# UzL-ITS/dash

Hardware: AMD Instinct MI355X
Metric: online garbled inferences/sec (MiniONN CIFAR-10 CNN) (higher is better)
Workload: dtype uint8 label components / int8 MFMA (exact modular arithmetic)

## Files before the change

### dash_amd/csrc/hip/gadget_common.h

```cpp
#pragma once

#include <cmath>
#include <cstdio>
#include <cstdlib>

#include "kargs.h"
#include "launch.h"

namespace dash {
namespace dev {

constexpr size_t kAesLds = 0;

#ifndef DASH_AES_BLOCK
#define DASH_AES_BLOCK 512
#endif
constexpr int kAesBlock = DASH_AES_BLOCK;
#ifndef DASH_AES_MINBLOCKS
#define DASH_AES_MINBLOCKS 6
#endif
constexpr int kAesMinBlocks = DASH_AES_MINBLOCKS;
#ifndef DASH_SA_MINBLOCKS
#define DASH_SA_MINBLOCKS 6
#endif
constexpr int kSignApproxMinWaves = DASH_SA_MINBLOCKS;
#ifndef DASH_SA_CHUNK
#define DASH_SA_CHUNK 16
#endif
constexpr int kSignApproxChunk = DASH_SA_CHUNK;

static int aes_block_cap(int bs) {
    const int waves = std::max(kAesMinBlocks, kSignApproxMinWaves);
    const int resident = std::max(1, std::min(waves * 256 / bs, 160 * 1024 / DASH_AES_LDS_BYTES));
    return 4 * resident * num_cus();
}
static inline dim3 grid_aes(int64_t n, int bs, int y, int z) {
    int64_t nx = (n + bs - 1) / bs;
    const int64_t capx = std::max<int64_t>(1, aes_block_cap(bs) / (static_cast<int64_t>(y) * z));
    return dim3(static_cast<unsigned>(std::min(nx, capx)), y, z);
}
static inline int aes_bs(int64_t n, int y, int z) {
    const int64_t lanes = n * y * z;
    int bs = kAesBlock;
    while (bs > 64 && lanes < static_cast<int64_t>(bs) * num_cus()) bs >>= 1;
    return bs;
}
struct LaunchDims {
    dim3 grid, block;
};
static inline LaunchDims aes_dims(const char* kernel, int64_t n, int y, int z) {
    const int bs = aes_bs(n, y, z);
    const LaunchDims d{grid_aes(n, bs, y, z), dim3(bs)};
    if (launch_log_on()) {
        std::string name(kernel);
        if (!name.empty() && name.front() == '(') name = name.substr(1, name.size() - 2);
        launch_log_add("aes." + name, d.grid, d.block);
    }
    return d;
}
#define AES_LAUNCH_GGL(kernel, n, y, z, lds, st, ...)                        \
    do {                                                                     \
        const LaunchDims d_ = aes_dims(#kernel, (n), (y), (z));              \
        hipLaunchKernelGGL(kernel, d_.grid, d_.block, lds, st, __VA_ARGS__); \
    } while (0)

#define AES_PROLOGUE(tab, rk)                    \
    __shared__ __attribute__((aligned(16))) uint32_t lds_aes[DASH_AES_LDS_WORDS]; \
    aes_lds_fill(lds_aes, tab);                   \
    const AesCtx aes = aes_ctx(lds_aes, rk)

template <int BS, int U, bool ZERO = false>
__device__ __forceinline__ void lds_stage_rows(uint8_t* S, const act_t* L, int64_t N, int64_t e0, int c0, int cnt) {
    constexpr int W = BS / 16;
    const int units = cnt * W;
    for (int x0 = threadIdx.x; x0 < units; x0 += U * BS) {
        uint4 v[U];
#pragma unroll
        for (int h = 0; h < U; ++h) {
            const int x = x0 + h * BS;
            const int64_t e = e0 + 16 * (x % W);
            if constexpr (ZERO) v[h] = make_uint4(0u, 0u, 0u, 0u);
            if (x < units && e < N) v[h] = *reinterpret_cast<const uint4*>(L + static_cast<int64_t>(c0 + x / W) * N + e);
        }
#pragma unroll
        for (int h = 0; h < U; ++h) {
            const int x = x0 + h * BS;
            if (x < units) *reinterpret_cast<uint4*>(S + (x / W) * BS + 16 * (x % W)) = v[h];
        }
    }
}
template <int BS>
__device__ __forceinline__ void lds_store_rows(act_t* L, const uint8_t* S, int64_t N, int64_t e0, int c0, int cnt) {
    constexpr int W = BS / 16;
    const int units = cnt * W;
    for (int x = threadIdx.x; x < units; x += BS) {
        const int64_t e = e0 + 16 * (x % W);
        if (e < N)
            *reinterpret_cast<uint4*>(L + static_cast<int64_t>(c0 + x / W) * N + e) =
                *reinterpret_cast<const uint4*>(S + (x / W) * BS + 16 * (x % W));
    }
}
static inline bool stage_ok(int64_t N, int bs) {
    static const bool on = [] {
        const char* e = std::getenv("DASH_MRS_STAGE");
        return !(e && e[0] == '0');
    }();
    return on && N % 16 == 0 && N >= bs;
}

#ifndef DASH_UA_MINBLOCKS
#define DASH_UA_MINBLOCKS 4
#endif

template <int CTRL>
__device__ __forceinline__ u128 dpp128(u128 v) {
    const uint32_t w0 = static_cast<uint32_t>(__builtin_amdgcn_mov_dpp(static_cast<int>(static_cast<uint32_t>(v)), CTRL, 0xF, 0xF, false));
    const uint32_t w1 = static_cast<uint32_t>(__builtin_amdgcn_mov_dpp(static_cast<int>(static_cast<uint32_t>(v >> 32)), CTRL, 0xF, 0xF, false));
    const uint32_t w2 = static_cast<uint32_t>(__builtin_amdgcn_mov_dpp(static_cast<int>(static_cast<uint32_t>(v >> 64)), CTRL, 0xF, 0xF, false));
    const uint32_t w3 = static_cast<uint32_t>(__builtin_amdgcn_mov_dpp(static_cast<int>(static_cast<uint32_t>(v >> 96)), CTRL, 0xF, 0xF, false));
    return (static_cast<u128>((static_cast<uint64_t>(w3) << 32) | w2) << 64) | ((static_cast<uint64_t>(w1) << 32) | w0);
}
__device__ __forceinline__ u128 quad_sum128(u128 v) {
    v += dpp128<0xB1>(v);
    return v + dpp128<0x4E>(v);
}
struct QPow {
    u128 d1, d2, d3, d4;
    __device__ __forceinline__ void init(const ModC& m) {
        d1 = static_cast<u128>(m.D);
        d2 = d1 * d1;
        d3 = d2 * d1;
        d4 = d2 * d2;
    }
    __device__ __forceinline__ u128 first(int g) const {
        return g == 0 ? static_cast<u128>(1) : (g == 1 ? d1 : (g == 2 ? d2 : d3));
    }
};

}
}
```

### dash_amd/csrc/hip/launch.h

```cpp
#pragma once

#include <hip/hip_runtime.h>

#include <algorithm>
#include <atomic>
#include <cstdlib>
#include <map>
#include <mutex>
#include <string>
#include <vector>

#include "kargs.h"

namespace dash {
namespace dev {

int num_cus();
void set_planning_cus(int n);
int planning_cus_override();
int64_t joint_fuse_min_elems();
int joint_fuse_mode();
void set_joint_fuse(int mode);
bool joint_fuse_pick(int64_t N, int B);
bool joint_fuse(int64_t N, int B);
bool leaky_fuse(int64_t N, int B);
bool clip_fuse_pick(int64_t N, int B);
bool clip_fuse(int64_t N, int B);
constexpr int kConstModDefault = 1;
int const_mod_mode();
void set_const_mod(int mode);
inline bool const_mod_on() { return const_mod_mode() >= 1; }
inline bool const_mod_chain() { return const_mod_mode() >= 2; }
void const_mod_count(bool chain);
long const_mod_launches(bool chain);
constexpr int kChainFpK = 7;
inline bool chain_const_mod_pick(const int* p, int k) {
    if (k != kChainFpK) return false;
    for (int r = 0; r < k; ++r)
        if (p[r] != static_cast<int>(kFirstPrimes[r])) return false;
    return true;
}
extern std::atomic<bool> g_launch_log_on;
inline bool launch_log_on() { return g_launch_log_on.load(std::memory_order_relaxed); }
void launch_log_enable(bool on);
void launch_log_add(const std::string& form, dim3 grid, dim3 block);
std::vector<std::string> launch_log_take();


void launch_sign_approx(const SignArgs& a, const Act& x, const ModC* mc, const AesGlobals& g, hipStream_t st);
void launch_sign_chain(const SignArgs& a, int maxn, const ModC* mc, const AesGlobals& g, hipStream_t st);
void launch_unpack(const u128* P, int nres, const Act& out, const CrtInfo& mods, const ModC* mc, int64_t N, int B,
                   hipStream_t st);
void launch_clip_hash(const ClipArgs& a, u128* hx, uint16_t* colx, const Act& x, int B, const ModC* mc,
                      const AesGlobals& g, hipStream_t st);
void launch_clip_sign_mrs(const MrsArgs& a, const Act& x, int B, const ModC* mc, const AesGlobals& g, hipStream_t st);
void launch_clip_mult(const ClipArgs& a, const Act& x, const Act& y, int B, const ModC* mc, hipStream_t st);
void launch_argmax_diff(const Act& v, const Act& d, int64_t P, int ops, int cnt, int pubq, const CrtInfo& crt, int B,
                        hipStream_t st);
void launch_argmax_hash(const Act& d, const CrtInfo& crt, int64_t N, u128* hx, uint16_t* colx, uint64_t gate0, int B,
                        const ModC* mc, const AesGlobals& g, hipStream_t st);
void launch_argmax_mult(const ArgMaxArgs& a, bool val, bool l0, const Act& v, const Act& d, const Act& i, const Act& ed,
                        const Act& nv, const Act& ni, int B, const ModC* mc, hipStream_t st);
void launch_pwl_key(const PwlArgs& a, u128* kx, uint16_t* colx, const Act& x, int B, const ModC* mc, hipStream_t st);
void launch_pwl_mult(const PwlArgs& a, const Act& x, const Act& y, int B, const ModC* mc, hipStream_t st);
void launch_leaky_mult(const SignArgs& a, const LeakyTab& lk, const Act& x, const Act& y, const u128* gtab,
                       const u128* etab, const ModC* mc, hipStream_t st);
void launch_leaky_mrs(const MrsArgs& a, const SignArgs& sa, const LeakyTab& lk, const Act& x, const Act& y,
                      const u128* gtab, const u128* etab, int B, const ModC* mc, const AesGlobals& g, hipStream_t st);
void launch_rescale_leaky_out(const MrsArgs& a, const SignArgs& sa, const LeakyTab& lk, const Act& x, const Act& y,
                              const u128* gtab, const u128* etab, int B, const ModC* mc, const AesGlobals& g,
                              hipStream_t st);
void launch_relu_mult(const SignArgs& a, const Act& x, const Act& y, const u128* gtab, const u128* etab,
                      const ModC* mc, hipStream_t st);
void launch_rescale_hash(const Act& x, int fi, int s, const int16_t* up, int up_stride, int add_up, int64_t N, int B,
                         u128* h0, uint16_t* col0, const ModC* mc, const AesGlobals& g, hipStream_t st, int hard = 0);
void launch_rescale_update(const RescaleArgs& a, const Act& x, int B, const ModC* mc, hipStream_t st);
void launch_rescale_post(const Act& x, const CrtInfo& crt, int64_t N, int B, const u128* signP, const int16_t* down,
                         int lab_stride, const int* lab_off, const ModC* mc, hipStream_t st);
void launch_rescale_hash_sign(const u128* signP, const u128* du, int64_t N, int B, u128* h0, uint16_t* col0,
                              const AesGlobals& g, hipStream_t st);
void launch_rescale_update_approx(const RescaleArgs& r, const SignArgs& a, const Act& x, const int16_t* delta,
                                  const u128* zh, int B, const ModC* mc, const AesGlobals& g, hipStream_t st);
void launch_rescale_mrs(const MrsArgs& a, const Act& x, int B, const ModC* mc, const AesGlobals& g, hipStream_t st,
                        bool chain_only = false);
void launch_rescale_mrs_out(const MrsArgs& a, const Act& x, int B, const ModC* mc, const AesGlobals& g,
                            hipStream_t st);
template <int K>
void launch_mrs_chain_k(const MrsArgs& a, const Act& x, int B, const ModC* mc, const AesGlobals& g, hipStream_t st);
void launch_rescale_relu_out(const MrsArgs& a, const SignArgs& sa, const Act& x, const Act& y, const u128* gtab,
                             const u128* etab, int B, const ModC* mc, const AesGlobals& g, hipStream_t st);
void launch_rescale_clip_out(const MrsArgs& a, const ClipArgs& ca, const Act& x, const Act& y, int B, const ModC* mc,
                             const AesGlobals& g, hipStream_t st);
void launch_relu_joint(const SignArgs& sa, const Act& x, const Act& y, const u128* gtab, const u128* etab, int B,
                       const ModC* mc, const AesGlobals& g, hipStream_t st);
void launch_relu_mrs(const MrsArgs& a, const SignArgs& sa, const Act& x, const Act& y, const u128* gtab,
                     const u128* etab, int B, const ModC* mc, const AesGlobals& g, hipStream_t st);
void launch_base_ext(const BEArgs& a, const Act& x, int B, const ModC* mc, const AesGlobals& g, hipStream_t st);
void launch_proj(const ProjArgs& a, const Act& x, const Act& y, int B, const ModC* mc, const AesGlobals& g,
                 hipStream_t st);
void launch_mul(const MulArgs& a, bool square, const Act& x, const Act& ys, const Act& y, int B, const ModC* mc,
                hipStream_t st);
void launch_label_key(const CrtInfo& crt, int64_t N, u128* kx, uint16_t* colx, const Act& x, int B, const ModC* mc,
                      hipStream_t st);
void launch_matmul(const MatMulArgs& a, const Act& y, int B, const ModC* mc, hipStream_t st);
void launch_mult(const MultArgs& a, const Act& x, const Act& y, int B, const ModC* mc, const AesGlobals& g,
                 hipStream_t st);

void launch_copy_gather(const Act& in, int64_t Nin, const Act& out, int64_t Nout, const int64_t* idx,
                        const CrtInfo& crt, int B, hipStream_t st);
void launch_gather(const Act& in, int64_t Nin, const Act& out, int64_t Nout, const int32_t* idx4, const int64_t* idx8,
                   const CrtInfo& crt, int B, hipStream_t st);
struct BilinearArgs {
    int C, H, W, OH, OW, OWp;
    const int2* rows;
    const int2* cols;
    const uint16_t* wrow;
    const uint16_t* wcol;
    uint32_t mq[kMaxRes];
};
struct BilinearTables {
    std::vector<int2> rows, cols;
    std::vector<uint16_t> wrow, wcol;
};
template <class Geom>
BilinearTables bilinear_tables(BilinearArgs& a, const Geom& G, const int* mods, int k) {
    a.C = static_cast<int>(G.C); a.H = static_cast<int>(G.H); a.W = static_cast<int>(G.W);
    a.OH = static_cast<int>(G.OH); a.OW = static_cast<int>(G.OW);
    a.OWp = (a.OW + 3) / 4 * 4;
    BilinearTables t;
    t.rows.resize(static_cast<size_t>(a.OH));
    t.cols.assign(static_cast<size_t>(a.OWp), make_int2(0, 0));
    t.wrow.resize(static_cast<size_t>(k) * a.OH);
    t.wcol.assign(static_cast<size_t>(k) * a.OWp, 0);
    for (int oy = 0; oy < a.OH; ++oy)
        t.rows[oy] = make_int2(static_cast<int>((*G.y0)[oy]), static_cast<int>((*G.y1)[oy]));
    for (int ox = 0; ox < a.OW; ++ox)
        t.cols[ox] = make_int2(static_cast<int>((*G.x0)[ox]), static_cast<int>((*G.x1)[ox]));
    for (int j = 0; j < k; ++j) {
        const int p = mods[j];
        a.mq[j] = static_cast<uint32_t>((uint64_t(1) << 32) / static_cast<uint64_t>(p));
        for (int oy = 0; oy < a.OH; ++oy)
            t.wrow[static_cast<size_t>(j) * a.OH + oy] = static_cast<uint16_t>(G.wy(oy, 0, p) | G.wy(oy, 1, p) << 8);
        for (int ox = 0; ox < a.OW; ++ox)
            t.wcol[static_cast<size_t>(j) * a.OWp + ox] = static_cast<uint16_t>(G.wx(ox, 0, p) | G.wx(ox, 1, p) << 8);
    }
    return t;
}
void launch_bilinear(const BilinearArgs& g, bool dword, const Act& in, const Act& out, const CrtInfo& crt, int B,
                     hipStream_t st);
void launch_pair_diff(const Act& v, int64_t Nv, const Act& d, int64_t Nout, int ops, int cnt, const CrtInfo& crt, int B,
                      hipStream_t st);
void launch_pair_add(const Act& v, int64_t Nv, const Act& r, const Act& nv, int64_t Nout, int ops, int cnt, int cnt1,
                     const CrtInfo& crt, int B, hipStream_t st);
void launch_add(const Act& x, const Act& y, int64_t N, const CrtInfo& crt, int B, hipStream_t st);
void launch_window_sum(const Act& in, int64_t Nin, const Act& out, int64_t Nout, const int64_t* idx, int K,
                       const CrtInfo& crt, int B, hipStream_t st);
struct PoolArgs {
    int C, H, W, kh, kw, sh, sw, ph, pw, OH, OW;
};
void launch_pool_sum(const Act& in, const Act& out, const PoolArgs& g, const CrtInfo& crt, int B, hipStream_t st);
void launch_concat_copy(const Act& src, int64_t Ns, const Act& out, int64_t Nout, int64_t off, const CrtInfo& crt,
                        int B, hipStream_t st);
void launch_aes_bench(u128* out, int blocks, int iters, const AesGlobals& g, hipStream_t st);
void launch_aes_test(const u128* in, u128* out, int64_t n, const AesGlobals& g, hipStream_t st);
void launch_hard_test(const u128* key, const uint64_t* gate, const uint32_t* sub, const uint32_t* blk, u128* out,
                      int64_t n, hipStream_t st);
constexpr int kModkTestRow = 64;
void launch_modk_test(int q, const uint32_t* r, int64_t N, uint32_t* out, hipStream_t st);
void launch_codec_test(const int16_t* labels, int64_t N, int q, const ModC* mc, u128* comp, int16_t* decomp,
                       hipStream_t st);

struct DenseArgs {
    CrtInfo crt;
    int64_t K, O;
    const int16_t* w[kMaxRes];
    const int32_t* zc[kMaxRes];
    const int16_t* bias[kMaxRes];
    const int16_t* zero;
    int lab_stride;
    int lab_off[kMaxRes];
    const int32_t* src;
// ... 300 lines not shown
```

### dash_amd/csrc/hip/mrs_chain.h

```cpp
#pragma once

#include "gadget_common.h"

namespace dash {
namespace dev {

__device__ __forceinline__ u128 add_packed(u128 a, u128 b, u128 hmask) {
    return ((a & ~hmask) + (b & ~hmask)) ^ ((a ^ b) & hmask);
}

#ifndef DASH_MRS_CHUNK
#define DASH_MRS_CHUNK 4
#endif
constexpr int kMrsChunk = DASH_MRS_CHUNK;
#ifndef DASH_MRS_M2CH
#define DASH_MRS_M2CH 16
#endif
template <int K>
__device__ __forceinline__ constexpr int mrs_pair(int l, int j) {
    return l * (2 * K - l - 1) / 2 + (j - l - 1);
}

template <int MODE>
__device__ __forceinline__ constexpr uint32_t mrs_row_sub(int i) {
    return tw_sub(MODE == 1 ? kTwSmrs : kTwMrs, static_cast<uint32_t>(i));
}
__device__ __forceinline__ void store_ypads(const MrsArgs& a, u128 key, int b, int64_t N, int64_t e) {
    const uint64_t g = a.rgate0 ^ static_cast<uint64_t>(e);
    for (int blk = 0; 4 * blk < a.ny; ++blk) {
        u128 p[4];
        hard_block(key, g, tw_sub(kTwMmy, 0), static_cast<uint32_t>(blk), p);
#pragma unroll
        for (int q = 0; q < 4; ++q)
            if (4 * blk + q < a.ny) a.ys[(static_cast<int64_t>(b) * a.ny + 4 * blk + q) * N + e] = p[q];
    }
}

template <int MODE>
__device__ __forceinline__ void store_sign_key(const MrsArgs& a, u128 key, int b, int64_t N, int64_t e) {
    if (MODE >= 1 && a.ks) a.ks[static_cast<int64_t>(b) * N + e] = key;
}

#ifndef DASH_CHAIN2_WAVES
#define DASH_CHAIN2_WAVES 4
#endif
template <int K, int MODE>
__global__ __launch_bounds__(kAesBlock, MODE == 2 ? DASH_CHAIN2_WAVES : DASH_UA_MINBLOCKS) void k_mrs_chain(MrsArgs a, Act x, const ModC* mc,
                                                                          const uint32_t* te0, const uint32_t* rk) {
    (void)te0;
    (void)rk;
    const int b = blockIdx.z;
    const int64_t N = a.N;
    constexpr int NP = K * (K - 1) / 2 > 0 ? K * (K - 1) / 2 : 1;
    for (int64_t e = static_cast<int64_t>(blockIdx.x) * blockDim.x + threadIdx.x; e < N;
         e += static_cast<int64_t>(gridDim.x) * blockDim.x) {
        const u128* row0 = a.tab + (static_cast<int64_t>(b) * N + e) * a.n_tab;
        u128* PS = a.ps + static_cast<int64_t>(b) * NP * N + e;
        u128 acc = 0;
#pragma unroll
        for (int i = 0; i < (MODE >= 1 ? K - 1 : K); ++i) {
            const int r = MODE >= 1 ? (i + 1) % K : i;
            const ModC m = mc[a.crt.p[r]];
            const int n = static_cast<int>(m.n);
            const act_t* L = x.p[r] + static_cast<int64_t>(b) * n * N + e;
            DigitStream ds[K > 1 ? K - 1 : 1];
#pragma unroll
            for (int l = 0; l < i; ++l) ds[l].init(PS[static_cast<int64_t>(mrs_pair<K>(l, i)) * N]);
            CompressFwd cf;
            cf.init();
            uint32_t col = 0;
            uint16_t cur[kMrsChunk], nxt[kMrsChunk];
#pragma unroll
            for (int u = 0; u < kMrsChunk; ++u)
                if (u < n) cur[u] = static_cast<uint16_t>(L[static_cast<int64_t>(u) * N]);
            for (int c0 = 0; c0 < n; c0 += kMrsChunk) {
#pragma unroll
                for (int u = 0; u < kMrsChunk; ++u)
                    if (c0 + kMrsChunk + u < n) nxt[u] = static_cast<uint16_t>(L[static_cast<int64_t>(c0 + kMrsChunk + u) * N]);
#pragma unroll
                for (int u = 0; u < kMrsChunk; ++u)
                    if (c0 + u < n) {
                        uint32_t d = cur[u];
#pragma unroll
                        for (int l = 0; l < i; ++l) {
                            const uint32_t s = ds[l].next(m);
                            d = d >= s ? d - s : d + m.q - s;
                        }
                        if (c0 + u == 0) col = d;
                        cf.push(d, m);
                    }
#pragma unroll
                for (int u = 0; u < kMrsChunk; ++u) cur[u] = nxt[u];
            }
            constexpr int kExtra = MODE == 1 ? 0 : 1;
            const int nt = K - 1 - i + kExtra;
            const u128* row = row0 + a.dig_off[i] + static_cast<int64_t>(col) * nt;
            u128 E[K];
#pragma unroll
            for (int t = 0; t < nt; ++t) E[t] = row[t];
            hard_unmask_n<K>(E, nt, cf.finish(), a.gate0 ^ static_cast<uint64_t>(e), mrs_row_sub<MODE>(i));
#pragma unroll
            for (int t = 0; t < K - 1 - i; ++t) PS[static_cast<int64_t>(mrs_pair<K>(i, i + 1 + t)) * N] = E[t];
            if (MODE != 1) acc = add_packed(acc, E[K - 1 - i], a.hmask);
        }
        if (MODE >= 1) {
            const ModC m = mc[a.crt.p[0]];
            const act_t* L = x.p[0] + static_cast<int64_t>(b) * m.n * N + e;
            u128 key = compress_cm<DASH_MRS_M2CH>(L, N, m);
#pragma unroll
            for (int l = 0; l < K - 1; ++l) key ^= PS[static_cast<int64_t>(mrs_pair<K>(l, K - 1)) * N];
            const uint32_t c = static_cast<uint32_t>(key) & 1u;
            u128 E = 0;
            if (MODE == 2)
                E = row0[a.dig_off[K - 1] + c] - hard_pad(key, a.gate0 ^ static_cast<uint64_t>(e), mrs_row_sub<MODE>(K - 1), 0);
            store_ypads(a, key, b, N, e);
            store_sign_key<MODE>(a, key, b, N, e);
            a.cs[static_cast<int64_t>(b) * N + e] = static_cast<uint8_t>(c);
            if (MODE == 2) acc = add_packed(acc, E, a.hmask);
        }
        if (MODE == 1) continue;
        const uint32_t col = static_cast<uint32_t>(acc) & static_cast<uint32_t>(a.T - 1);
        const u128* row = row0 + a.fin_off + static_cast<int64_t>(col) * K;
        u128 F[K];
#pragma unroll
        for (int j = 0; j < K; ++j) F[j] = row[j];
        hard_unmask<K>(F, acc, a.gate0 ^ static_cast<uint64_t>(e), mrs_row_sub<0>(K));
#pragma unroll
        for (int j = 0; j < K; ++j) a.pf[(static_cast<int64_t>(b) * K + j) * N + e] = F[j];
    }
}

constexpr int kMrsBS = 512;
#ifndef DASH_CHAIN_LDS_SLOTS
#define DASH_CHAIN_LDS_SLOTS 1
#endif
constexpr int kChainSlots = DASH_CHAIN_LDS_SLOTS;
#ifndef DASH_CHAIN_FOLD
#define DASH_CHAIN_FOLD 1
#endif
constexpr bool kChainFold = DASH_CHAIN_FOLD != 0;
#ifndef DASH_MRS_CAP
#define DASH_MRS_CAP (DASH_CHAIN_LDS_SLOTS > 6 ? 32 : 64)
#endif
constexpr int kMrsCap = DASH_MRS_CAP;
constexpr int kChainLds = kChainSlots * 16 * kMrsBS + kMrsCap * kMrsBS;
static_assert(kChainSlots >= 0 && kChainSlots * 16 * kMrsBS <= (64 << 10), "slot offsets are instruction immediates (16 bits)");
static_assert(kChainLds <= (80 << 10), "two staged-chain blocks per CU: at most 80 KiB of LDS each");
static_assert(kMrsCap >= 20 && kMrsCap % 4 == 0, "a staging pass holds whole chunks: m.c <= 20 (p = 3)");

constexpr int kPsHbm = -1;
constexpr int kPsFold = -2;
constexpr int kPsNone = -3;
constexpr int chain_pair_idx(int K, int l, int j) { return l * (2 * K - l - 1) / 2 + (j - l - 1); }
template <int K>
struct ChainSlotMap {
    int slot[K * (K - 1) / 2 > 0 ? K * (K - 1) / 2 : 1];
};
template <int K, int MODE, int S>
constexpr ChainSlotMap<K> chain_slot_map() {
    ChainSlotMap<K> r{};
    constexpr int jmax = MODE >= 1 && kChainFold ? K - 2 : K - 1;
    int live[K + 1] = {};
    for (int l = 0; l < K; ++l)
        for (int j = l + 1; j < K; ++j) {
            const int p = chain_pair_idx(K, l, j);
            if (j > jmax) r.slot[p] = kPsFold;
            else if (S <= 0) r.slot[p] = kPsHbm;
            else {
                r.slot[p] = kPsNone;
                for (int t = l; t < j; ++t) ++live[t];
            }
        }
    while (true) {
        int tp = 0;
        for (int t = 1; t < K; ++t)
            if (live[t] > live[tp]) tp = t;
        if (live[tp] <= S) break;
        int bl = -1, bj = -1;
        for (int l = 0; l <= tp; ++l)
            for (int j = tp + 1; j <= jmax; ++j)
                if (r.slot[chain_pair_idx(K, l, j)] == kPsNone && (bl < 0 || j - l > bj - bl)) bl = l, bj = j;
        r.slot[chain_pair_idx(K, bl, bj)] = kPsHbm;
        for (int t = bl; t < bj; ++t) --live[t];
    }
    int busy_to[S > 0 ? S : 1] = {};
    for (int l = 0; l < K; ++l)
        for (int j = l + 1; j <= jmax; ++j) {
            const int p = chain_pair_idx(K, l, j);
            if (r.slot[p] != kPsNone) continue;
            for (int s = 0; s < S; ++s)
                if (busy_to[s] <= l) {
                    r.slot[p] = s;
                    busy_to[s] = j;
                    break;
                }
        }
    return r;
}
template <int K, int MODE, int S>
constexpr bool chain_slot_map_ok() {
    const ChainSlotMap<K> m = chain_slot_map<K, MODE, S>();
    for (int l = 0; l < K; ++l)
        for (int j = l + 1; j < K; ++j) {
            const int s = m.slot[chain_pair_idx(K, l, j)];
            if (MODE >= 1 && kChainFold && j == K - 1) {
                if (s != kPsFold) return false;
                continue;
            }
            if (s != kPsHbm && (s < 0 || s >= S)) return false;
            if (s < 0) continue;
            for (int l2 = 0; l2 < K; ++l2)
                for (int j2 = l2 + 1; j2 < K; ++j2)
                    if ((l2 != l || j2 != j) && m.slot[chain_pair_idx(K, l2, j2)] == s && l < j2 && l2 < j) return false;
        }
    return true;
}
template <int S, int... Ks>
constexpr bool chain_slot_maps_ok() {
    return ((chain_slot_map_ok<Ks, 0, S>() && chain_slot_map_ok<Ks, 1, S>() && chain_slot_map_ok<Ks, 2, S>()) && ...);
}
static_assert(chain_slot_maps_ok<kChainSlots, 2, 3, 4, 5, 6, 7, 8, 9, 10, 11, 12>(), "pair slot map (build's slot count)");
static_assert(chain_slot_maps_ok<6, 2, 3, 4, 5, 6, 7, 8, 9, 10, 11, 12>() && chain_slot_maps_ok<8, 2, 3, 4, 5, 6, 7, 8, 9, 10, 11, 12>() &&
                  chain_slot_maps_ok<1, 2, 3, 4, 5, 6, 7, 8, 9, 10, 11, 12>() && chain_slot_maps_ok<0, 2, 3, 4, 5, 6, 7, 8, 9, 10, 11, 12>(),
              "pair slot map (the measured slot counts, one slot, none)");
static_assert(!kChainFold ||
                  (chain_slot_map<7, 2, 6>().slot[chain_pair_idx(7, 0, 4)] == kPsHbm && chain_slot_map<7, 2, 6>().slot[chain_pair_idx(7, 0, 5)] == kPsHbm &&
                   chain_slot_map<7, 2, 6>().slot[chain_pair_idx(7, 1, 5)] == kPsHbm && chain_slot_map<7, 2, 6>().slot[chain_pair_idx(7, 0, 3)] >= 0),
              "K = 7 joint chain: the three longest-lived pairs overflow");
template <int K, int MODE>
struct ChainSlotsOf {
    static constexpr ChainSlotMap<K> map = chain_slot_map<K, MODE, kChainSlots>();
};
template <int K, int MODE, int I, int T = 0, int NT>
__device__ __forceinline__ void chain_s_put(const u128 (&E)[NT], u128* PS, u128* psl, int64_t N, bool valid, u128& sx) {
    if constexpr (T < K - 1 - I) {
        constexpr int p = chain_pair_idx(K, I, I + 1 + T);
        constexpr int s = ChainSlotsOf<K, MODE>::map.slot[p];
        if constexpr (s == kPsFold) {
            uint64_t lo = static_cast<uint64_t>(sx ^ E[T]), hi = static_cast<uint64_t>((sx ^ E[T]) >> 64);
            asm("" : "+v"(lo), "+v"(hi));
            sx = (static_cast<u128>(hi) << 64) | lo;
        } else if constexpr (s >= 0) psl[s * kMrsBS] = E[T];
        else if (valid) PS[static_cast<int64_t>(p) * N] = E[T];
        chain_s_put<K, MODE, I, T + 1>(E, PS, psl, N, valid, sx);
    }
}
template <int K, int MODE, int I, bool LDS, int L = 0, int NQ>
__device__ __forceinline__ void chain_s_get(u128 (&Q)[NQ], const u128* PS, const u128* psl, int64_t N) {
    if constexpr (L < I) {
        constexpr int p = chain_pair_idx(K, L, I);
        constexpr int s = ChainSlotsOf<K, MODE>::map.slot[p];
        static_assert(s != kPsFold && s != kPsNone, "a folded pair has no reader");
        if constexpr (LDS && s >= 0) Q[L] = psl[s * kMrsBS];
        if constexpr (!LDS && s < 0) Q[L] = PS[static_cast<int64_t>(p) * N];
        chain_s_get<K, MODE, I, LDS, L + 1>(Q, PS, psl, N);
    }
}
#ifndef DASH_STAGE_U
#define DASH_STAGE_U 2
#endif
constexpr int kStageU = DASH_STAGE_U;
#ifndef DASH_STAGE_RD
#define DASH_STAGE_RD 4
#endif
constexpr int kStageRd = DASH_STAGE_RD;
template <class MK, int I, int CNT>
__device__ __forceinline__ uint32_t chain_chunk_k(const uint8_t* sc, bool valid, uint32_t (&rr)[I > 0 ? I : 1], uint32_t& d0) {
    typename MK::template Acc<CNT> acc;
    static_for<0, (CNT + 1) / 2>([&](auto tt) __attribute__((always_inline)) {
        constexpr int t = 2 * decltype(tt)::value;
        constexpr bool two = t + 1 < CNT;
        uint32_t s0 = 0, s1 = 0;
        static_for<0, I>([&](auto ll) __attribute__((always_inline)) {
            constexpr int l = decltype(ll)::value;
            uint32_t a0, a1 = 0;
            if constexpr (two) MK::digit2(rr[l], a0, a1);
            else a0 = MK::digit(rr[l]);
            s0 += a0;
            s1 += a1;
        });
        uint32_t da = valid ? sc[t * kMrsBS] : 0u;
        if constexpr (I > 0) da = MK::template mod<(I + 1) * MK::q>(da + I * MK::q - s0);
        if constexpr (t == 0) d0 = da;
        acc.template push<t>(da);
        if constexpr (two) {
            uint32_t db = valid ? sc[(t + 1) * kMrsBS] : 0u;
            if constexpr (I > 0) db = MK::template mod<(I + 1) * MK::q>(db + I * MK::q - s1);
            acc.template push<t + 1>(db);
        }
        pair_fence();
    });
    return acc.value();
}
template <int K, int MODE, int I, bool FP = false>
__device__ __forceinline__ void chain_s_pos(const MrsArgs& a, uint64_t gate, const ModC* mc, const Act& x,
                                            uint8_t* stg, int b, int64_t N, int64_t e0, int tid, bool valid,
                                            const u128* row0, u128* PS, u128* psl, u128& acc, u128& sx) {
    constexpr int kLast = MODE >= 1 ? K - 1 : K;
    constexpr int NQ = I > 0 ? I : 1;
    if constexpr (I < kLast) {
        constexpr int i = I;
        {
            constexpr int r = MODE >= 1 ? (i + 1) % K : i;
            const ModC m = mc[a.crt.p[r]];
            const int n = static_cast<int>(m.n);
            const act_t* L = x.p[r] + static_cast<int64_t>(b) * n * N;
            uint32_t col = 0;
            u128 key;
            constexpr int kExtra = MODE == 1 ? 0 : 1;
            constexpr int nt = K - 1 - i + kExtra;
            u128 pf0 = 0, pf1 = 0;
            if constexpr (r == 0) {
                u128 Q[NQ];
                chain_s_get<K, MODE, I, false>(Q, PS, psl, N);
                chain_s_get<K, MODE, I, true>(Q, PS, psl, N);
                DigitStream ds[NQ];
#pragma unroll
                for (int l = 0; l < i; ++l) ds[l].init(Q[l]);
                CompressFwd cf;
                cf.init();
                for (int c0 = 0; c0 < n; c0 += kMrsCap) {
                    const int cnt = min(kMrsCap, n - c0);
                    __syncthreads();
                    lds_stage_rows<kMrsBS, kStageU, true>(stg, L, N, e0, c0, cnt);
                    __syncthreads();
                    for (int c = 0; c < cnt; ++c) {
                        uint32_t d = valid ? stg[c * kMrsBS + tid] : 0u;
#pragma unroll
                        for (int l = 0; l < i; ++l) {
                            const uint32_t s = ds[l].next(m);
                            d = d >= s ? d - s : d + m.q - s;
                        }
                        if (c0 + c == 0) {
                            col = d;
                            const u128* rowp = row0 + a.dig_off[i] + static_cast<int64_t>(col) * nt;
                            pf0 = rowp[0];
                            pf1 = rowp[nt - 1];
                        }
                        cf.push(d, m);
                    }
                }
                key = cf.finish();
            } else if constexpr (FP) {
                using MK = ModK<kFirstPrimes[r]>;
                constexpr int mcn = static_cast<int>(MK::c), nk = static_cast<int>(MK::n);
                constexpr int PC = kMrsCap / mcn, nfull = nk / mcn, tail = nk % mcn;
                static_assert(nfull >= 1 && PC >= 1, "a label holds a whole chunk, and so does a staging pass");
                u128 Q[NQ];
                chain_s_get<K, MODE, I, false>(Q, PS, psl, N);
                u128 C = 0, PW = 1;
#pragma unroll 1
                for (int ch0 = 0; ch0 * mcn < nk; ch0 += PC) {
                    const int p0 = ch0 * mcn, pcnt = min(PC * mcn, nk - p0);
                    __syncthreads();
                    lds_stage_rows<kMrsBS, kStageU, true>(stg, L, N, e0, p0, pcnt);
                    __syncthreads();
                    if (ch0 == 0) chain_s_get<K, MODE, I, true>(Q, PS, psl, N);
                    const int fe = min(ch0 + PC, nfull);
#pragma unroll 1
                    for (int ch = ch0; ch < fe; ++ch) {
                        uint32_t rr[NQ];
#pragma unroll
                        for (int l = 0; l < i; ++l) rr[l] = MK::divmod(Q[l]);
                        uint32_t d0 = 0;
                        const uint32_t v = chain_chunk_k<MK, I, mcn>(stg + (ch - ch0) * mcn * kMrsBS + tid, valid, rr, d0);
                        if (ch == 0) {
                            col = d0;
                            const u128* rowp = row0 + a.dig_off[i] + static_cast<int64_t>(col) * nt;
                            pf0 = rowp[0];
                            pf1 = rowp[nt - 1];
                        }
                        C += PW * static_cast<u128>(v);
                        PW *= static_cast<u128>(MK::D);
                    }
                    if constexpr (tail > 0) {
                        if (nfull < ch0 + PC) {
                            uint32_t rr[NQ];
#pragma unroll
                            for (int l = 0; l < i; ++l) rr[l] = MK::divmod(Q[l]);
                            uint32_t d0 = 0;
                            C += PW * static_cast<u128>(chain_chunk_k<MK, I, tail>(stg + (nfull - ch0) * mcn * kMrsBS + tid, valid, rr, d0));
                        }
                    }
                }
                key = C;
            } else {
                u128 Q[NQ];
                chain_s_get<K, MODE, I, false>(Q, PS, psl, N);
                u128 C = 0, PW = 1;
                const int mcn = static_cast<int>(m.c);
                const int pass = kMrsCap / mcn * mcn;
                for (int p0 = 0; p0 < n; p0 += pass) {
                    const int pcnt = min(pass, n - p0);
                    __syncthreads();
                    lds_stage_rows<kMrsBS, kStageU, true>(stg, L, N, e0, p0, pcnt);
                    __syncthreads();
                    if (p0 == 0) chain_s_get<K, MODE, I, true>(Q, PS, psl, N);
                    for (int c0 = 0; c0 < pcnt; c0 += mcn) {
                        uint32_t rr[NQ];
#pragma unroll
                        for (int l = 0; l < i; ++l) rr[l] = divmod128(Q[l], m);
                        const int cnt = min(mcn, pcnt - c0);
                        uint32_t v = 0, pt = 1;
                        auto digit = [&](int t) -> uint32_t {
                            uint32_t d = valid ? stg[(c0 + t) * kMrsBS + tid] : 0u;
#pragma unroll
                            for (int l = 0; l < i; ++l) {
                                const uint32_t sd = chunk_digit(rr[l], m);
                                d = d >= sd ? d - sd : d + m.q - sd;
                            }
                            return d;
                        };
                        int t0 = 0;
                        if (p0 + c0 == 0) {
                            const uint32_t d = digit(0);
                            col = d;
                            const u128* rowp = row0 + a.dig_off[i] + static_cast<int64_t>(col) * nt;
                            pf0 = rowp[0];
                            pf1 = rowp[nt - 1];
                            v = d;
                            pt = m.q;
                            t0 = 1;
                        }
#pragma unroll 2
                        for (int t = t0; t < cnt; ++t) {
                            const uint32_t d = digit(t);
                            v += d * pt;
                            pt *= m.q;
                        }
                        C += PW * static_cast<u128>(v);
                        PW *= static_cast<u128>(m.D);
                    }
                }
                key = C;
            }
            const u128* row = row0 + a.dig_off[i] + static_cast<int64_t>(col) * nt;
            u128 E[nt];
            E[0] = pf0;
#pragma unroll
            for (int t = 1; t < nt - 1; ++t) E[t] = row[t];
            if constexpr (nt > 1) E[nt - 1] = pf1;
            hard_unmask<nt>(E, key, gate, mrs_row_sub<MODE>(i));
            chain_s_put<K, MODE, I>(E, PS, psl, N, valid, sx);
            if constexpr (MODE != 1) acc = add_packed(acc, E[K - 1 - i], a.hmask);
        }
        chain_s_pos<K, MODE, I + 1, FP>(a, gate, mc, x, stg, b, N, e0, tid, valid, row0, PS, psl, acc, sx);
    }
}

template <int K, int MODE, bool FP = false>
__global__ __launch_bounds__(kMrsBS, MODE == 2 ? DASH_CHAIN2_WAVES : DASH_UA_MINBLOCKS) void k_mrs_chain_s(
    MrsArgs a, Act x, const ModC* mc, const uint32_t* te0, const uint32_t* rk) {
    (void)te0;
    (void)rk;
    __shared__ __attribute__((aligned(16))) uint8_t lds[kChainLds];
    const int b = blockIdx.z;
    const int64_t N = a.N;
    constexpr int NP = K * (K - 1) / 2 > 0 ? K * (K - 1) / 2 : 1;
    const int tid = static_cast<int>(threadIdx.x);
    u128* psl = reinterpret_cast<u128*>(lds) + tid;
    uint8_t* stg = lds + kChainSlots * 16 * kMrsBS;
    for (int64_t e0 = static_cast<int64_t>(blockIdx.x) * kMrsBS; e0 < N; e0 += static_cast<int64_t>(gridDim.x) * kMrsBS) {
        const bool valid = e0 + tid < N;
        const int64_t e = valid ? e0 + tid : N - 1;
        const u128* row0 = a.tab + (static_cast<int64_t>(b) * N + e) * a.n_tab;
        u128* PS = a.ps + static_cast<int64_t>(b) * NP * N + e;
        u128 acc = 0;
        u128 sx = 0;
        const uint64_t gate = a.gate0 ^ static_cast<uint64_t>(e);
        chain_s_pos<K, MODE, 0, FP>(a, gate, mc, x, stg, b, N, e0, tid, valid, row0, PS, psl, acc, sx);
        if (MODE >= 1) {
            const ModC m = mc[a.crt.p[0]];
            const int n = static_cast<int>(m.n);
            const act_t* L = x.p[0] + static_cast<int64_t>(b) * n * N;
            CompressFwd cf;
            cf.init();
            u128 kb = 0;
            for (int c0 = 0; c0 < n; c0 += kMrsCap) {
                const int cnt = min(kMrsCap, n - c0);
                __syncthreads();
                lds_stage_rows<kMrsBS, kStageU, true>(stg, L, N, e0, c0, cnt);
                __syncthreads();
                if (m.bits == 1) {
                    for (int w0 = 0; w0 < cnt; w0 += 32) {
                        uint32_t w = 0;
#pragma unroll 8
                        for (int u = 0; u < 32; ++u)
                            if (w0 + u < cnt) w |= (valid ? static_cast<uint32_t>(stg[(w0 + u) * kMrsBS + tid]) : 0u) << u;
                        kb |= static_cast<u128>(w) << (c0 + w0);
                    }
                } else {
                    for (int c = 0; c < cnt; ++c) cf.push(valid ? stg[c * kMrsBS + tid] : 0u, m);
                }
            }
            u128 key = m.bits == 1 ? kb : cf.finish();
            if constexpr (kChainFold) {
                key ^= sx;
            } else {
                u128 Q[K > 1 ? K - 1 : 1];
                chain_s_get<K, MODE, K - 1, false>(Q, PS, psl, N);
                chain_s_get<K, MODE, K - 1, true>(Q, PS, psl, N);
#pragma unroll
                for (int l = 0; l < K - 1; ++l) key ^= Q[l];
            }
            const uint32_t c = static_cast<uint32_t>(key) & 1u;
            u128 E = 0;
            if (MODE == 2) E = row0[a.dig_off[K - 1] + c] - hard_pad(key, gate, mrs_row_sub<MODE>(K - 1), 0);
            if (valid) {
                store_ypads(a, key, b, N, e);
                store_sign_key<MODE>(a, key, b, N, e);
                a.cs[static_cast<int64_t>(b) * N + e] = static_cast<uint8_t>(c);
            }
            if (MODE == 2) acc = add_packed(acc, E, a.hmask);
        }
        if (MODE == 1) continue;
        const uint32_t colf = static_cast<uint32_t>(acc) & static_cast<uint32_t>(a.T - 1);
        const u128* row = row0 + a.fin_off + static_cast<int64_t>(colf) * K;
        u128 F[K];
#pragma unroll
        for (int j = 0; j < K; ++j) F[j] = row[j];
        hard_unmask<K>(F, acc, gate, mrs_row_sub<0>(K));
        if (valid) {
#pragma unroll
            for (int j = 0; j < K; ++j) a.pf[(static_cast<int64_t>(b) * K + j) * N + e] = F[j];
        }
    }
}

constexpr int kMrsWBS = 256;
constexpr int kWaveU = 8;
template <int K, int MODE, int I>
__device__ __forceinline__ void chain_w_pos(const MrsArgs& a, uint64_t gate, const ModC* mc, const uint8_t* wst,
                                            const int* roff, int tid, bool valid, const u128* row0, u128* PS,
                                            u128& acc) {
    constexpr int kLast = MODE >= 1 ? K - 1 : K;
    if constexpr (I < kLast) {
        constexpr int r = MODE >= 1 ? (I + 1) % K : I;
        const ModC m = mc[a.crt.p[r]];
        const int n = static_cast<int>(m.n);
        const uint8_t* Ls = wst + roff[r] * kMrsWBS + tid;
        uint32_t col = 0;
        u128 key;
        constexpr int kExtra = MODE == 1 ? 0 : 1;
        constexpr int nt = K - 1 - I + kExtra;
        u128 pf0 = 0, pf1 = 0;
        if constexpr (r == 0) {
            DigitStream ds[I > 0 ? I : 1];
#pragma unroll
            for (int l = 0; l < I; ++l) ds[l].init(PS[mrs_pair<K>(l, I)]);
            CompressFwd cf;
            cf.init();
            for (int c = 0; c < n; ++c) {
                uint32_t d = valid ? Ls[c * kMrsWBS] : 0u;
#pragma unroll
                for (int l = 0; l < I; ++l) {
                    const uint32_t s = ds[l].next(m);
                    d = d >= s ? d - s : d + m.q - s;
                }
                if (c == 0) {
                    col = d;
                    const u128* rowp = row0 + a.dig_off[I] + static_cast<int64_t>(col) * nt;
                    pf0 = rowp[0];
                    pf1 = rowp[nt - 1];
                }
                cf.push(d, m);
            }
            key = cf.finish();
        } else {
            u128 Q[I > 0 ? I : 1];
#pragma unroll
            for (int l = 0; l < I; ++l) Q[l] = PS[mrs_pair<K>(l, I)];
            u128 C = 0, PW = 1;
            for (int c0 = 0; c0 < n; c0 += static_cast<int>(m.c)) {
                uint32_t rr[I > 0 ? I : 1];
#pragma unroll
                for (int l = 0; l < I; ++l) rr[l] = divmod128(Q[l], m);
                const int cnt = min(static_cast<int>(m.c), n - c0);
                uint32_t v = 0, pt = 1;
                for (int t = 0; t < cnt; ++t) {
                    uint32_t d = valid ? Ls[(c0 + t) * kMrsWBS] : 0u;
#pragma unroll
                    for (int l = 0; l < I; ++l) {
                        const uint32_t sd = chunk_digit(rr[l], m);
                        d = d >= sd ? d - sd : d + m.q - sd;
                    }
                    if (c0 + t == 0) {
                        col = d;
                        const u128* rowp = row0 + a.dig_off[I] + static_cast<int64_t>(col) * nt;
                        pf0 = rowp[0];
                        pf1 = rowp[nt - 1];
                    }
                    v += d * pt;
                    pt *= m.q;
                }
                C += PW * static_cast<u128>(v);
                PW *= static_cast<u128>(m.D);
            }
            key = C;
        }
        const u128* row = row0 + a.dig_off[I] + static_cast<int64_t>(col) * nt;
        u128 E[nt > 0 ? nt : 1];
        E[0] = pf0;
#pragma unroll
        for (int t = 1; t < nt - 1; ++t) E[t] = row[t];
        if constexpr (nt > 1) E[nt - 1] = pf1;
        if constexpr (nt > 0) hard_unmask<nt>(E, key, gate, mrs_row_sub<MODE>(I));
#pragma unroll
        for (int t = 0; t < K - 1 - I; ++t) PS[mrs_pair<K>(I, I + 1 + t)] = E[t];
        if constexpr (MODE != 1) acc = add_packed(acc, E[K - 1 - I], a.hmask);
        chain_w_pos<K, MODE, I + 1>(a, gate, mc, wst, roff, tid, valid, row0, PS, acc);
    }
}

template <int K, int MODE>
__global__ __launch_bounds__(kMrsWBS, 1) void k_mrs_chain_w(MrsArgs a, Act x, const ModC* mc, const uint32_t* te0,
                                                            const uint32_t* rk) {
    (void)te0;
    (void)rk;
    extern __shared__ __attribute__((aligned(16))) uint8_t wst[];
    const int b = blockIdx.z;
    const int64_t N = a.N;
    constexpr int NP = K * (K - 1) / 2 > 0 ? K * (K - 1) / 2 : 1;
    const int tid = static_cast<int>(threadIdx.x);
    int roff[K + 1];
    const act_t* src[K];
    roff[0] = 0;
#pragma unroll
    for (int r = 0; r < K; ++r) {
        const int n = static_cast<int>(mc[a.crt.p[r]].n);
        roff[r + 1] = roff[r] + n;
        src[r] = x.p[r] + static_cast<int64_t>(b) * n * N;
    }
    const int units = roff[K] * (kMrsWBS / 16);
    for (int64_t e0 = static_cast<int64_t>(blockIdx.x) * kMrsWBS; e0 < N; e0 += static_cast<int64_t>(gridDim.x) * kMrsWBS) {
        __syncthreads();
        if (N % 16 != 0) {
            constexpr int kWaveBU = 32;
            const int bunits = roff[K] * kMrsWBS;
            const int64_t e = e0 + tid;
            for (int x0 = tid; x0 < bunits; x0 += kWaveBU * kMrsWBS) {
                uint32_t v[kWaveBU];
#pragma unroll
                for (int h = 0; h < kWaveBU; ++h) {
                    const int xu = x0 + h * kMrsWBS;
                    const int g = xu / kMrsWBS;
// ... 580 lines not shown
```

Baseline: 4125.

## Double-buffer chain staging with async global-to-LDS DMA and default to chained const-mod

Replaces the synchronous two-barrier staging of label rows into LDS in the staged MRS chain kernel with a double-buffered pipeline. It uses global_load_lds to prefetch the next fill, including the next residue or the next grid-stride tile, while the current fill is consumed. A compile-time checker verifies that the fill schedule alternates halves and covers every row. Separately, the default const-mod mode is raised from 1 to 2, which enables the chained constant-modulus path. The pipeline halves the rows per fill, adding more waits, and adds vmcnt waits and LDS pressure in exchange for overlapping HBM latency with compute.

```diff
diff --git a/dash_amd/csrc/hip/gadget_common.h b/dash_amd/csrc/hip/gadget_common.h
--- a/dash_amd/csrc/hip/gadget_common.h
+++ b/dash_amd/csrc/hip/gadget_common.h
@@ -89,6 +89,24 @@
         }
     }
 }
+template <int BS, int MAXR>
+__device__ __forceinline__ void lds_dma_rows(uint8_t* S, const act_t* L, int64_t N, int64_t e0, int c0, int cnt) {
+    static_assert(BS % 64 == 0 && sizeof(act_t) == 1, "whole waves, byte labels");
+    constexpr int W = BS / 16;
+    const int units = cnt * W;
+    int t0 = static_cast<int>(threadIdx.x);
+    asm volatile("" : "+v"(t0));
+    const int lane = t0 & 63;
+#pragma unroll
+    for (int h = 0; h < (MAXR * W + BS - 1) / BS; ++h) {
+        const int x = t0 + h * BS;
+        const int64_t e = e0 + 16 * (x % W);
+        if (x < units && e < N)
+            __builtin_amdgcn_global_load_lds(
+                (const __attribute__((address_space(1))) void*)(L + static_cast<int64_t>(c0 + x / W) * N + e),
+                (__attribute__((address_space(3))) void*)(S + (x - lane) * 16), 16, 0, 0);
+    }
+}
 template <int BS>
 __device__ __forceinline__ void lds_store_rows(act_t* L, const uint8_t* S, int64_t N, int64_t e0, int c0, int cnt) {
     constexpr int W = BS / 16;
diff --git a/dash_amd/csrc/hip/launch.h b/dash_amd/csrc/hip/launch.h
--- a/dash_amd/csrc/hip/launch.h
+++ b/dash_amd/csrc/hip/launch.h
@@ -26,7 +26,7 @@
 bool leaky_fuse(int64_t N, int B);
 bool clip_fuse_pick(int64_t N, int B);
 bool clip_fuse(int64_t N, int B);
-constexpr int kConstModDefault = 1;
+constexpr int kConstModDefault = 2;
 int const_mod_mode();
 void set_const_mod(int mode);
 inline bool const_mod_on() { return const_mod_mode() >= 1; }
diff --git a/dash_amd/csrc/hip/mrs_chain.h b/dash_amd/csrc/hip/mrs_chain.h
--- a/dash_amd/csrc/hip/mrs_chain.h
+++ b/dash_amd/csrc/hip/mrs_chain.h
@@ -143,10 +143,21 @@
 #define DASH_MRS_CAP (DASH_CHAIN_LDS_SLOTS > 6 ? 32 : 64)
 #endif
 constexpr int kMrsCap = DASH_MRS_CAP;
-constexpr int kChainLds = kChainSlots * 16 * kMrsBS + kMrsCap * kMrsBS;
+#ifndef DASH_CHAIN_PIPE
+#define DASH_CHAIN_PIPE 1
+#endif
+constexpr bool kChainPipe = DASH_CHAIN_PIPE != 0;
+#ifndef DASH_CHAIN_PIPE_ROWS
+#define DASH_CHAIN_PIPE_ROWS (DASH_MRS_CAP / 2)
+#endif
+constexpr int kFillRows = kChainPipe ? DASH_CHAIN_PIPE_ROWS : kMrsCap;
+constexpr int kFillBytes = kFillRows * kMrsBS;
+constexpr int kChainLds = kChainSlots * 16 * kMrsBS + (kChainPipe ? 2 : 1) * kFillBytes;
 static_assert(kChainSlots >= 0 && kChainSlots * 16 * kMrsBS <= (64 << 10), "slot offsets are instruction immediates (16 bits)");
 static_assert(kChainLds <= (80 << 10), "two staged-chain blocks per CU: at most 80 KiB of LDS each");
 static_assert(kMrsCap >= 20 && kMrsCap % 4 == 0, "a staging pass holds whole chunks: m.c <= 20 (p = 3)");
+static_assert(kFillRows >= 20 && kFillRows % 2 == 0, "a fill holds whole chunks (m.c <= 20, p = 3) and whole 1 KiB wave writes (two rows)");
+static_assert(kFillBytes % 1024 == 0 && (kChainSlots * 16 * kMrsBS) % 1024 == 0, "no wave write crosses from one half into the other");
 
 constexpr int kPsHbm = -1;
 constexpr int kPsFold = -2;
@@ -264,6 +275,110 @@
 #define DASH_STAGE_RD 4
 #endif
 constexpr int kStageRd = DASH_STAGE_RD;
+constexpr int chain_fill_res(int K, int mode, int P) { return mode >= 1 ? (P + 1) % K : P; }
+constexpr int chain_fill_step(int c) { return kFillRows / c * c; }
+constexpr bool chain_fill_schedule_ok(int K, int mode) {
+    int seen[12][128] = {};
+    int t = 0, last_half = 1;
+    for (int tile = 0; tile < 2; ++tile)
+        for (int P = 0; P < K; ++P) {
+            const int r = chain_fill_res(K, mode, P);
+            const int q = static_cast<int>(kFirstPrimes[r]);
+            const int n = r == 0 ? 128 : static_cast<int>(modk_n(q));
+            const int step = chain_fill_step(r == 0 ? 1 : static_cast<int>(modk_c(q)));
+            if (step < 1 || step > kFillRows || (r != 0 && step % static_cast<int>(modk_c(q)) != 0)) return false;
+            for (int f = 0; f * step < n; ++f, ++t) {
+                const int c0 = f * step, cnt = n - c0 < step ? n - c0 : step;
+                if (cnt < 1 || cnt > kFillRows) return false;
+                const int half = kChainPipe ? t & 1 : 0;
+                if (kChainPipe && half == last_half) return false;
+                last_half = half;
+                for (int c = c0; c < c0 + cnt; ++c) ++seen[r][c];
+            }
+        }
+    for (int r = 0; r < K; ++r) {
+        const int n = r == 0 ? 128 : static_cast<int>(modk_n(kFirstPrimes[r]));
+        for (int c = 0; c < 128; ++c)
+            if (seen[r][c] != (c < n ? 2 : 0)) return false;
+    }
+    return true;
+}
+template <int... Ks>
+constexpr bool chain_fill_schedules_ok() {
+    return ((chain_fill_schedule_ok(Ks, 0) && chain_fill_schedule_ok(Ks, 1) && chain_fill_schedule_ok(Ks, 2)) && ...);
+}
+static_assert(chain_fill_schedules_ok<2, 3, 4, 5, 6, 7, 8, 9, 10, 11, 12>(), "fill schedule of the staged chain");
+
+template <int K>
+struct ChainFillInfo {
+    uint32_t v[K];
+    __device__ __forceinline__ void init(const MrsArgs& a, const ModC* mc) {
+#pragma unroll
+        for (int r = 0; r < K; ++r) {
+            const ModC m = mc[a.crt.p[r]];
+            v[r] = m.n | static_cast<uint32_t>(r == 0 ? kFillRows : chain_fill_step(static_cast<int>(m.c))) << 8;
+        }
+    }
+};
+template <int K, int MODE, int P, bool FP>
+__device__ __forceinline__ void chain_fill_src(const ChainFillInfo<K>& fi, const Act& x, int b, int64_t N,
+                                               const act_t*& L, int& n, int& step) {
+    constexpr int r = chain_fill_res(K, MODE, P);
+    if constexpr (FP && r != 0) {
+        using MK = ModK<kFirstPrimes[r]>;
+        n = static_cast<int>(MK::n);
+        step = chain_fill_step(static_cast<int>(MK::c));
+    } else {
+        n = static_cast<int>(fi.v[r] & 0xffu);
+        step = static_cast<int>(fi.v[r] >> 8);
+    }
+    L = x.p[r] + static_cast<int64_t>(b) * n * N;
+}
+template <int K, int MODE, int P, bool FP>
+__device__ __forceinline__ void chain_fill_first(const ChainFillInfo<K>& fi, const Act& x, uint8_t* dst, int b,
+                                                 int64_t N, int64_t e0) {
+    const act_t* L;
+    int n, step;
+    chain_fill_src<K, MODE, P, FP>(fi, x, b, N, L, n, step);
+    lds_dma_rows<kMrsBS, kFillRows>(dst, L, N, e0, 0, min(step, n));
+}
+template <int K, int MODE, int P, bool FP>
+__device__ __forceinline__ const uint8_t* chain_fill_wait(const ChainFillInfo<K>& fi, const Act& x, uint8_t* stg, int b,
+                                                          int64_t N, int64_t e0, int f, int& t) {
+    if constexpr (!kChainPipe) {
+        const act_t* L;
+        int n, step;
+        chain_fill_src<K, MODE, P, FP>(fi, x, b, N, L, n, step);
+        __syncthreads();
+        lds_stage_rows<kMrsBS, kStageU, true>(stg, L, N, e0, f * step, min(step, n - f * step));
+        __syncthreads();
+        return stg;
+    } else {
+        asm volatile("s_waitcnt vmcnt(0)" ::: "memory");
+        __syncthreads();
+        const uint8_t* cur = stg + (t & 1) * kFillBytes;
+        ++t;
+        return cur;
+    }
+}
+template <int K, int MODE, int P, bool FP>
+__device__ __forceinline__ void chain_fill_issue(const ChainFillInfo<K>& fi, const Act& x, uint8_t* stg, int b,
+                                                 int64_t N, int64_t e0, int f, int t) {
+    if constexpr (kChainPipe) {
+        const act_t* L;
+        int n, step;
+        chain_fill_src<K, MODE, P, FP>(fi, x, b, N, L, n, step);
+        uint8_t* nxt = stg + (t & 1) * kFillBytes;
+        const int c1 = (f + 1) * step;
+        if (c1 < n) lds_dma_rows<kMrsBS, kFillRows>(nxt, L, N, e0, c1, min(step, n - c1));
+        else if constexpr (P + 1 < K) chain_fill_first<K, MODE, P + 1, FP>(fi, x, nxt, b, N, e0);
+        else {
+            const int64_t e1 = e0 + static_cast<int64_t>(gridDim.x) * kMrsBS;
+            if (e1 < N) chain_fill_first<K, MODE, 0, FP>(fi, x, nxt, b, N, e1);
+        }
+    }
+}
+
 template <class MK, int I, int CNT>
 __device__ __forceinline__ uint32_t chain_chunk_k(const uint8_t* sc, bool valid, uint32_t (&rr)[I > 0 ? I : 1], uint32_t& d0) {
     typename MK::template Acc<CNT> acc;
@@ -294,7 +409,7 @@
 }
 template <int K, int MODE, int I, bool FP = false>
 __device__ __forceinline__ void chain_s_pos(const MrsArgs& a, uint64_t gate, const ModC* mc, const Act& x,
-                                            uint8_t* stg, int b, int64_t N, int64_t e0, int tid, bool valid,
+                                            uint8_t* stg, const ChainFillInfo<K>& fi, int& ft, int b, int64_t N, int64_t e0, int tid, bool valid,
                                             const u128* row0, u128* PS, u128* psl, u128& acc, u128& sx) {
     constexpr int kLast = MODE >= 1 ? K - 1 : K;
     constexpr int NQ = I > 0 ? I : 1;
@@ -304,7 +419,6 @@
             constexpr int r = MODE >= 1 ? (i + 1) % K : i;
             const ModC m = mc[a.crt.p[r]];
             const int n = static_cast<int>(m.n);
-            const act_t* L = x.p[r] + static_cast<int64_t>(b) * n * N;
             uint32_t col = 0;
             u128 key;
             constexpr int kExtra = MODE == 1 ? 0 : 1;
@@ -319,13 +433,11 @@
                 for (int l = 0; l < i; ++l) ds[l].init(Q[l]);
                 CompressFwd cf;
                 cf.init();
-                for (int c0 = 0; c0 < n; c0 += kMrsCap) {
-                    const int cnt = min(kMrsCap, n - c0);
-                    __syncthreads();
-                    lds_stage_rows<kMrsBS, kStageU, true>(stg, L, N, e0, c0, cnt);
-                    __syncthreads();
+                for (int c0 = 0, f = 0; c0 < n; c0 += kFillRows, ++f) {
+                    const int cnt = min(kFillRows, n - c0);
+                    const uint8_t* img = chain_fill_wait<K, MODE, I, FP>(fi, x, stg, b, N, e0, f, ft) + tid;
                     for (int c = 0; c < cnt; ++c) {
-                        uint32_t d = valid ? stg[c * kMrsBS + tid] : 0u;
+                        uint32_t d = valid ? img[c * kMrsBS] : 0u;
 #pragma unroll
                         for (int l = 0; l < i; ++l) {
                             const uint32_t s = ds[l].next(m);
@@ -337,6 +449,7 @@
                             pf0 = rowp[0];
                             pf1 = rowp[nt - 1];
                         }
+                        if (c == 0) chain_fill_issue<K, MODE, I, FP>(fi, x, stg, b, N, e0, f, ft);
                         cf.push(d, m);
                     }
                 }
@@ -344,17 +457,14 @@
             } else if constexpr (FP) {
                 using MK = ModK<kFirstPrimes[r]>;
                 constexpr int mcn = static_cast<int>(MK::c), nk = static_cast<int>(MK::n);
-                constexpr int PC = kMrsCap / mcn, nfull = nk / mcn, tail = nk % mcn;
-                static_assert(nfull >= 1 && PC >= 1, "a label holds a whole chunk, and so does a staging pass");
+                constexpr int PC = kFillRows / mcn, nfull = nk / mcn, tail = nk % mcn;
+                static_assert(nfull >= 1 && PC >= 1, "a label holds a whole chunk, and so does a fill");
                 u128 Q[NQ];
                 chain_s_get<K, MODE, I, false>(Q, PS, psl, N);
                 u128 C = 0, PW = 1;
 #pragma unroll 1
-                for (int ch0 = 0; ch0 * mcn < nk; ch0 += PC) {
-                    const int p0 = ch0 * mcn, pcnt = min(PC * mcn, nk - p0);
-                    __syncthreads();
-                    lds_stage_rows<kMrsBS, kStageU, true>(stg, L, N, e0, p0, pcnt);
-                    __syncthreads();
+                for (int ch0 = 0, f = 0; ch0 * mcn < nk; ch0 += PC, ++f) {
+                    const uint8_t* img = chain_fill_wait<K, MODE, I, FP>(fi, x, stg, b, N, e0, f, ft) + tid;
                     if (ch0 == 0) chain_s_get<K, MODE, I, true>(Q, PS, psl, N);
                     const int fe = min(ch0 + PC, nfull);
 #pragma unroll 1
@@ -363,23 +473,25 @@
 #pragma unroll
                         for (int l = 0; l < i; ++l) rr[l] = MK::divmod(Q[l]);
                         uint32_t d0 = 0;
-                        const uint32_t v = chain_chunk_k<MK, I, mcn>(stg + (ch - ch0) * mcn * kMrsBS + tid, valid, rr, d0);
+                        const uint32_t v = chain_chunk_k<MK, I, mcn>(img + (ch - ch0) * mcn * kMrsBS, valid, rr, d0);
                         if (ch == 0) {
                             col = d0;
                             const u128* rowp = row0 + a.dig_off[i] + static_cast<int64_t>(col) * nt;
                             pf0 = rowp[0];
                             pf1 = rowp[nt - 1];
                         }
+                        if (ch == ch0) chain_fill_issue<K, MODE, I, FP>(fi, x, stg, b, N, e0, f, ft);
                         C += PW * static_cast<u128>(v);
                         PW *= static_cast<u128>(MK::D);
                     }
+                    if (fe <= ch0) chain_fill_issue<K, MODE, I, FP>(fi, x, stg, b, N, e0, f, ft);
                     if constexpr (tail > 0) {
                         if (nfull < ch0 + PC) {
                             uint32_t rr[NQ];
 #pragma unroll
                             for (int l = 0; l < i; ++l) rr[l] = MK::divmod(Q[l]);
                             uint32_t d0 = 0;
-                            C += PW * static_cast<u128>(chain_chunk_k<MK, I, tail>(stg + (nfull - ch0) * mcn * kMrsBS + tid, valid, rr, d0));
+                            C += PW * static_cast<u128>(chain_chunk_k<MK, I, tail>(img + (nfull - ch0) * mcn * kMrsBS, valid, rr, d0));
                         }
                     }
                 }
@@ -389,12 +501,10 @@
                 chain_s_get<K, MODE, I, false>(Q, PS, psl, N);
                 u128 C = 0, PW = 1;
                 const int mcn = static_cast<int>(m.c);
-                const int pass = kMrsCap / mcn * mcn;
-                for (int p0 = 0; p0 < n; p0 += pass) {
+                const int pass = chain_fill_step(mcn);
+                for (int p0 = 0, f = 0; p0 < n; p0 += pass, ++f) {
                     const int pcnt = min(pass, n - p0);
-                    __syncthreads();
-                    lds_stage_rows<kMrsBS, kStageU, true>(stg, L, N, e0, p0, pcnt);
-                    __syncthreads();
+                    const uint8_t* img = chain_fill_wait<K, MODE, I, FP>(fi, x, stg, b, N, e0, f, ft) + tid;
                     if (p0 == 0) chain_s_get<K, MODE, I, true>(Q, PS, psl, N);
                     for (int c0 = 0; c0 < pcnt; c0 += mcn) {
                         uint32_t rr[NQ];
@@ -403,7 +513,7 @@
                         const int cnt = min(mcn, pcnt - c0);
                         uint32_t v = 0, pt = 1;
                         auto digit = [&](int t) -> uint32_t {
-                            uint32_t d = valid ? stg[(c0 + t) * kMrsBS + tid] : 0u;
+                            uint32_t d = valid ? img[(c0 + t) * kMrsBS] : 0u;
 #pragma unroll
                             for (int l = 0; l < i; ++l) {
                                 const uint32_t sd = chunk_digit(rr[l], m);
@@ -422,6 +532,7 @@
                             pt = m.q;
                             t0 = 1;
                         }
+                        if (c0 == 0) chain_fill_issue<K, MODE, I, FP>(fi, x, stg, b, N, e0, f, ft);
 #pragma unroll 2
                         for (int t = t0; t < cnt; ++t) {
                             const uint32_t d = digit(t);
@@ -444,7 +555,7 @@
             chain_s_put<K, MODE, I>(E, PS, psl, N, valid, sx);
             if constexpr (MODE != 1) acc = add_packed(acc, E[K - 1 - i], a.hmask);
         }
-        chain_s_pos<K, MODE, I + 1, FP>(a, gate, mc, x, stg, b, N, e0, tid, valid, row0, PS, psl, acc, sx);
+        chain_s_pos<K, MODE, I + 1, FP>(a, gate, mc, x, stg, fi, ft, b, N, e0, tid, valid, row0, PS, psl, acc, sx);
     }
 }
 
@@ -460,6 +571,13 @@
     const int tid = static_cast<int>(threadIdx.x);
     u128* psl = reinterpret_cast<u128*>(lds) + tid;
     uint8_t* stg = lds + kChainSlots * 16 * kMrsBS;
+    ChainFillInfo<K> fi;
+    fi.init(a, mc);
+    int ft = 0;
+    if constexpr (kChainPipe) {
+        if (static_cast<int64_t>(blockIdx.x) * kMrsBS < N)
+            chain_fill_first<K, MODE, 0, FP>(fi, x, stg, b, N, static_cast<int64_t>(blockIdx.x) * kMrsBS);
+    }
     for (int64_t e0 = static_cast<int64_t>(blockIdx.x) * kMrsBS; e0 < N; e0 += static_cast<int64_t>(gridDim.x) * kMrsBS) {
         const bool valid = e0 + tid < N;
         const int64_t e = valid ? e0 + tid : N - 1;
@@ -468,29 +586,27 @@
         u128 acc = 0;
         u128 sx = 0;
         const uint64_t gate = a.gate0 ^ static_cast<uint64_t>(e);
-        chain_s_pos<K, MODE, 0, FP>(a, gate, mc, x, stg, b, N, e0, tid, valid, row0, PS, psl, acc, sx);
+        chain_s_pos<K, MODE, 0, FP>(a, gate, mc, x, stg, fi, ft, b, N, e0, tid, valid, row0, PS, psl, acc, sx);
         if (MODE >= 1) {
             const ModC m = mc[a.crt.p[0]];
             const int n = static_cast<int>(m.n);
-            const act_t* L = x.p[0] + static_cast<int64_t>(b) * n * N;
             CompressFwd cf;
             cf.init();
             u128 kb = 0;
-            for (int c0 = 0; c0 < n; c0 += kMrsCap) {
-                const int cnt = min(kMrsCap, n - c0);
-                __syncthreads();
-                lds_stage_rows<kMrsBS, kStageU, true>(stg, L, N, e0, c0, cnt);
-                __syncthreads();
+            for (int c0 = 0, f = 0; c0 < n; c0 += kFillRows, ++f) {
+                const int cnt = min(kFillRows, n - c0);
+                const uint8_t* img = chain_fill_wait<K, MODE, K - 1, FP>(fi, x, stg, b, N, e0, f, ft) + tid;
+                chain_fill_issue<K, MODE, K - 1, FP>(fi, x, stg, b, N, e0, f, ft);
                 if (m.bits == 1) {
                     for (int w0 = 0; w0 < cnt; w0 += 32) {
                         uint32_t w = 0;
 #pragma unroll 8
                         for (int u = 0; u < 32; ++u)
-                            if (w0 + u < cnt) w |= (valid ? static_cast<uint32_t>(stg[(w0 + u) * kMrsBS + tid]) : 0u) << u;
+                            if (w0 + u < cnt) w |= (valid ? static_cast<uint32_t>(img[(w0 + u) * kMrsBS]) : 0u) << u;
                         kb |= static_cast<u128>(w) << (c0 + w0);
                     }
                 } else {
-                    for (int c = 0; c < cnt; ++c) cf.push(valid ? stg[c * kMrsBS + tid] : 0u, m);
+                    for (int c = 0; c < cnt; ++c) cf.push(valid ? img[c * kMrsBS] : 0u, m);
                 }
             }
             u128 key = m.bits == 1 ? kb : cf.finish();
```

Measured after the change: 4216 (median of 6 runs). 2.2% higher.
